# QMC-Cornell/sqmc

Measured on AMD Instinct MI355X. Metric: walker-steps/sec, higher is better.
Workload: dtype f64; 1 GPU; C2 cc-pVDZ r=1.24253 (8e,26o, D2h) semistochastic walk, uniform2 proposal, w_abs_gen_target=100000, size_deterministic=1000, Psi_T 100 dets, tau_multiplier 0.1, min_wt 0.5, r_initiator 1; rng=counter, parallelism=single GPU, devices=1, chained_runs=True

## Files before the change

### sqmc_amd/csrc/bucket_kernels.h

```cpp
#pragma once

__global__ void __launch_bounds__(BK_T) k_bucket_boundaries(const u64 *__restrict__ keys, long long n0, BucketArgs ba) { bk_rebalance_block(ba, keys, n0); }
__global__ void __launch_bounds__(BK_T) k_bucket_partition(const u64 *__restrict__ keys, long long n0, long long nch, u64 invalid_key, BucketArgs ba, int n_extra) {
  if ((int)blockIdx.x < n_extra) { bk_rebalance_block(ba, keys, n0); return; }
  __shared__ u32 spl[BK_MAXB];
  __shared__ u32 wcnt[BK_T / 64][BK_MAXB];
  const long long blk = (long long)blockIdx.x - n_extra;
  const long long c = blk * BK_T + threadIdx.x;
  u64 word = 0; u32 key = 0; bool valid = false;
  if (c < nch) word = keys[n0 + c];
  bucket_partition_stage(spl, &wcnt[0][0], BK_MAXB, keys, n0, ba);
  if (c < nch) { key = (u32)(word >> 32); valid = (u64)key != invalid_key; }
  __syncthreads();
  bucket_partition_block(spl, &wcnt[0][0], BK_MAXB, valid, key, word, blk, ba);
}

__device__ __forceinline__ void bk_fold(double &wt, int &ini, int &d, double w2, u32 fs, const StepP &p) {
  const int i2 = flg_init(fs), d2 = flg_impd(fs);
  const bool same_sign = (w2 * wt > 0);
  if (same_sign) { if (i2 > ini) ini = i2; }
  if (d == -2) { if (d2 == 0) d = 0; }
  else if (d2 == -2) { if (d != 0) d = -2; }
  else if (d != 0 && d != -2) { const int a_ = d2 < 0 ? -d2 : d2; if (a_ < d) d = a_; }
  if (!same_sign) {
    if (fabs(wt) < fabs(w2)) { if (ini != 3 || p.r_init == -1.0) ini = i2; }
    else if (fabs(wt) == fabs(w2)) { if (ini != 3 || p.r_init == -1.0) ini = 0; }
  }
  if (!(d == 0 && d2 == -1)) wt = wt + w2;
}

#ifdef BUCKET_PROF
__device__ unsigned long long g_bprof[16 * 1024];
#define BPROF(K) do { if (threadIdx.x == 0 && b < 1024) g_bprof[b * 16 + (K)] = wall_clock64(); } while (0)
#define BPROF_VAL(K, V) do { if (threadIdx.x == 0 && b < 1024) g_bprof[b * 16 + (K)] = (unsigned long long)(V); } while (0)
extern "C" int sqmc_gpu_debug_bprof(unsigned long long *out) { return (int)hipMemcpyFromSymbol(out, HIP_SYMBOL(g_bprof), sizeof(g_bprof)); }
#else
#define BPROF(K)
#define BPROF_VAL(K, V)
#endif
__device__ __forceinline__ u64 bk_block_excl_scan(u64 v, u64 *total) {
  __shared__ u64 wsum[BK_AT / 64];
  const int lane = threadIdx.x & 63, wv = threadIdx.x >> 6;
  const u64 inc = wave_incl_scan_u64(v, lane);
  if (lane == 63) wsum[wv] = inc;
  __syncthreads();
  u64 off = 0, tot = 0;
#pragma unroll
  for (int i = 0; i < BK_AT / 64; i++) { if (i < wv) off += wsum[i]; tot += wsum[i]; }
  __syncthreads();
  *total = tot;
  return off + inc - v;
}
__device__ __forceinline__ u64 bk_lookback_wide(u64 *__restrict__ state, int b, u64 tot) {
  __shared__ int s_pstar[BK_AT / 64]; __shared__ u64 s_part[BK_AT / 64];
  const int tid = threadIdx.x, lane = tid & 63, wv = tid >> 6;
  if (b == 0) { if (tid == 0) atomicExch((unsigned long long *)&state[0], SCAN_ST_INC | tot); return 0; }
  if (tid == 0) atomicExch((unsigned long long *)&state[b], SCAN_ST_AGG | tot);
  u64 w_[BK_MAXB / BK_AT]; int ix_[BK_MAXB / BK_AT];
  int pstar = -1;
#pragma unroll
  for (int q = 0; q < BK_MAXB / BK_AT; q++) {
    const int idx = b - 1 - tid - q * BK_AT; ix_[q] = idx; w_[q] = 0;
    if (idx >= 0) {
      u64 w;
      do { w = atomicAdd((unsigned long long *)&state[idx], 0ull); } while ((w >> 62) == 0);
      w_[q] = w;
      if ((w >> 62) == 2 && idx > pstar) pstar = idx;
    }
  }
  for (int o = 32; o > 0; o >>= 1) { const int x = __shfl_xor(pstar, o, 64); pstar = x > pstar ? x : pstar; }
  if (lane == 0) s_pstar[wv] = pstar;
  __syncthreads();
#pragma unroll
  for (int v = 0; v < BK_AT / 64; v++) pstar = s_pstar[v] > pstar ? s_pstar[v] : pstar;
  u64 sum = 0;
#pragma unroll
  for (int q = 0; q < BK_MAXB / BK_AT; q++) if (ix_[q] >= 0 && ix_[q] >= pstar) sum += w_[q] & SCAN_VAL_MASK;
  for (int o = 32; o > 0; o >>= 1) sum += __shfl_xor(sum, o, 64);
  if (lane == 0) s_part[wv] = sum;
  __syncthreads();
  u64 excl = 0;
#pragma unroll
  for (int v = 0; v < BK_AT / 64; v++) excl += s_part[v];
  if (tid == 0) atomicExch((unsigned long long *)&state[b], SCAN_ST_INC | (excl + tot));
  return excl;
}
#define BK_LONG_RUN 24
#define BK_LONG_MAX 32
#define BK_HQ_DETS (BK_CAP_T * 2 / 16)
template <int CTRL, int ROWMASK>
__device__ __forceinline__ double bk_dpp_f64(double v) {
  int lo = __double2loint(v), hi = __double2hiint(v);
  lo = __builtin_amdgcn_update_dpp(0, lo, CTRL, ROWMASK, 0xf, true);
  hi = __builtin_amdgcn_update_dpp(0, hi, CTRL, ROWMASK, 0xf, true);
  return __hiloint2double(hi, lo);
}
__device__ __forceinline__ double bk_wave_sum_lane63(double v) {
  v += bk_dpp_f64<0x111, 0xf>(v); v += bk_dpp_f64<0x112, 0xf>(v); v += bk_dpp_f64<0x114, 0xf>(v); v += bk_dpp_f64<0x118, 0xf>(v);
  v += bk_dpp_f64<0x142, 0xa>(v);
  v += bk_dpp_f64<0x143, 0xc>(v);
  return v;
}
#define BK_PER_ROWS ((BK_CAP_ROWS + BK_AT - 1) / BK_AT)
#define BK_PER_S ((BK_CAP_S + BK_AT - 1) / BK_AT)
#define BK_PER_R ((BK_CAP_R + BK_AT - 1) / BK_AT)
#define BK_PER_T ((BK_CAP_T + BK_AT - 1) / BK_AT)

__global__ void __launch_bounds__(BK_AT, BK_PER_CU * (BK_AT / 64) / 4) k_anneal_bucket(WalkArr w, WalkArr o, const u64 *__restrict__ rkeys, int *__restrict__ loc_imp,
                                                         const u64 *__restrict__ hkey, const u32 *__restrict__ hidx, u64 hmask,
                                                         const double *__restrict__ cnum, const double *__restrict__ cden,
                                                         double *__restrict__ partials, double *__restrict__ wabs_part, long long n0, long long nch, StepP p,
                                                         u64 invalid_key, u64 seed, u64 step, DevScalars *sc, BucketArgs ba, GateOut go, FusedSide fs, ChemDev dev) {
  __shared__ u64 sw[BK_CAP_S], sw2[BK_CAP_S];
  __shared__ u32 rk[BK_CAP_R];
  __shared__ double s_w[BK_CAP_T]; __shared__ u32 s_f[BK_CAP_T];
  __shared__ u32 m2s[BK_CAP_T];
  __shared__ __align__(16) unsigned short rnk[BK_CAP_T];
  constexpr int BK_SCR_TAB = (BK_CAP_T + 3) & ~3;
  constexpr int BK_SCR_ROWS = (BK_CAP_ROWS / 2 + 4) + BK_CAP_ROWS + 1, BK_SCR_CNT = (BK_AT / 64) * 1024 * (int)sizeof(bk_cnt_t) / 4, BK_SCR_TABEND = BK_SCR_TAB + ((int)sizeof(ChemTab) + 3) / 4;
  constexpr int BK_SCR_WORDS = ((BK_SCR_ROWS > BK_SCR_CNT ? (BK_SCR_ROWS > BK_SCR_TABEND ? BK_SCR_ROWS : BK_SCR_TABEND) : (BK_SCR_CNT > BK_SCR_TABEND ? BK_SCR_CNT : BK_SCR_TABEND)) + 3) & ~3;
  __shared__ __align__(16) u32 scratch[BK_SCR_WORDS];
  __shared__ unsigned short s_hq[BK_CAP_T]; __shared__ int s_hqn;
  static_assert(BK_CAP_T <= 4096 && (sizeof(bk_cnt_t) == 4 || BK_CAP_S <= 65535), "ranks inside a bucket are 12 bits; the counters hold a bucket's spawns");
  ChemTab *s_tab = (ChemTab *)(scratch + BK_SCR_TAB);
  u64 *s_hdet = (u64 *)rnk;
  __shared__ u32 s_tile; __shared__ u32 s_kmin, s_kmax;
  __shared__ double s_red[BK_AT / 64][NSTAT + 2];
  const int tid = threadIdx.x, lane = tid & 63, wv = tid >> 6;
  if (tid == 0) { s_tile = atomicAdd(ba.ticket, 1u); s_hqn = 0; }
  __syncthreads();
  const int b = (int)s_tile, B = ba.B, nsb = ba.nsb;
  const long long r_lo = bk_bound(ba, b, n0), r_hi = bk_bound(ba, b + 1, n0);
  const int R = (int)(r_hi - r_lo);
  BPROF(0);
  if (tid == 0) s_kmin = b ? (ba.kb ? ba.kb[b] : (u32)(rkeys[r_lo] >> 32)) : 0u;
  if (tid == 64) s_kmax = (b + 1 < B) ? (ba.kb ? ba.kb[b + 1] : (u32)(rkeys[r_hi] >> 32)) - 1u : (u32)invalid_key;
  unsigned short *seg_lo = (unsigned short *)scratch; u32 *seg_base = scratch + (BK_CAP_ROWS / 2 + 4);
  bool fits = nsb <= BK_CAP_ROWS && R <= BK_CAP_R && !(ba.kb && (b == 0 || b == B - 1) && R == 0);
  u32 rk_reg[BK_PER_R];
#pragma unroll
  for (int q = 0; q < BK_PER_R; q++) { const int i = tid + q * BK_AT; rk_reg[q] = (fits && i < R) ? (u32)(rkeys[r_lo + i] >> 32) : 0u; }
  int S = 0;
  const bool rows_ok = nsb <= BK_CAP_ROWS;
  if (rows_ok) {
    const int C = (nsb + BK_AT - 1) / BK_AT;
    unsigned short lo_[BK_PER_ROWS], hi_[BK_PER_ROWS];
#pragma unroll
    for (int q = 0; q < BK_PER_ROWS; q++) {
      const int t = tid * C + q;
      lo_[q] = 0; hi_[q] = 0;
      if (q < C && t < nsb) { const unsigned short *rp = ba.segoff + (long long)t * (B + 1) + b; lo_[q] = rp[0]; hi_[q] = rp[1]; }
    }
    u64 mine = 0;
#pragma unroll
    for (int q = 0; q < BK_PER_ROWS; q++) mine += (u64)(hi_[q] - lo_[q]);
    u64 tot; u32 ex = (u32)bk_block_excl_scan(mine, &tot);
#pragma unroll
    for (int q = 0; q < BK_PER_ROWS; q++) {
      const int t = tid * C + q;
      if (q < C && t < nsb) { seg_lo[t] = lo_[q]; seg_base[t] = ex; ex += (u32)(hi_[q] - lo_[q]); }
    }
    if (tid == 0) seg_base[nsb] = (u32)tot;
    S = (int)tot;
    fits = fits && S <= BK_CAP_S && R + S <= BK_CAP_T && !ba.force_retry;
  }
  const int T = R + S;
  if (!fits) {
    if (tid == 0) atomicExch((int *)&sc->retry, 1);
    if (tid == 0 && ba.scount && rows_ok) { ba.scount[b] = (u32)S; if (b == 0) ba.scount[B] = (u32)n0; }
#ifdef BUCKET_PROF
    if (tid == 0) printf("bucket %d of %d does not fit: rows %d, R %d, S %d (r_lo %lld)\n", b, B, nsb, R, S, r_lo);
#endif
    if (tid < 64) lookback_exclusive(ba.state, (u32)b, 0ull, tid);
    return;
  }
#pragma unroll
  for (int q = 0; q < BK_PER_R; q++) { const int i = tid + q * BK_AT; if (i < R) rk[i] = rk_reg[q]; }
  __syncthreads();
  BPROF(1);
  {
    u64 wv_[BK_PER_S];
#pragma unroll
    for (int q = 0; q < BK_PER_S; q++) {
      const int j = tid + q * BK_AT;
      wv_[q] = 0;
      if (j < S) {
        int lo = 0, hi = nsb;
        while (hi - lo > 1) { const int mid = (lo + hi) >> 1; if (seg_base[mid] <= (u32)j) lo = mid; else hi = mid; }
        wv_[q] = ba.words[(long long)lo * BK_T + seg_lo[lo] + ((u32)j - seg_base[lo])];
      }
    }
#pragma unroll
    for (int q = 0; q < BK_PER_S; q++) { const int j = tid + q * BK_AT; if (j < S) sw[j] = wv_[q]; }
  }
  __syncthreads();
  BPROF(2); BPROF_VAL(12, S); BPROF_VAL(13, R);
  if (tid == 0 && ba.scount) { ba.scount[b] = (u32)S; if (b == 0) ba.scount[B] = (u32)n0; }
  u64 *sa = sw, *sb = sw2;
  const bool gap_sort = R <= 1023;
  unsigned short *gs = (unsigned short *)m2s, *gst = gs + BK_CAP_S;
  static_assert((BK_CAP_S + 1026) * 2 <= BK_CAP_T * 4, "gap tables fit the merged-order array");
  if (gap_sort) {
    unsigned short *gp = s_hq;
    bk_cnt_t(*wcnt)[1024] = (bk_cnt_t(*)[1024])scratch;
    const u64 lt = (lane == 0) ? 0ull : (~0ull >> (64 - lane));
    const int chunk = ((S + BK_AT - 1) / BK_AT) * 64;
    for (int d = tid; d < BK_SCR_CNT; d += BK_AT) scratch[d] = 0;
    for (int j = tid; j < S; j += BK_AT) {
      const u32 k = (u32)(sa[j] >> 32);
      int lo = 0, hi = R;
      while (lo < hi) { const int mid = (lo + hi) >> 1; if (rk[mid] <= k) lo = mid + 1; else hi = mid; }
      gp[j] = (unsigned short)lo;
    }
    __syncthreads();
    {
      const int beg = wv * chunk, end = (beg + chunk < S) ? beg + chunk : S;
      for (int base = beg; base < end; base += 64) {
        const int idx = base + lane; const bool valid = idx < end;
        const u32 dig = valid ? (u32)gp[idx] : 0u;
        u64 same = __ballot(valid);
#pragma unroll
        for (int q = 0; q < 10; q++) { const u64 m = __ballot((dig >> q) & 1); same &= ((dig >> q) & 1) ? m : ~m; }
        const u32 rank = (u32)__popcll(same & lt), cnt = (u32)__popcll(same);
        u32 prev = 0;
        if (valid) prev = wcnt[wv][dig];
        __builtin_amdgcn_wave_barrier();
        if (valid && rank == 0) wcnt[wv][dig] = (bk_cnt_t)(prev + cnt);
        __builtin_amdgcn_wave_barrier();
        if (valid) rnk[idx] = (unsigned short)(prev + rank);
      }
    }
    __syncthreads();
    {
      u32 t2[2]; u64 sum = 0;
#pragma unroll
      for (int q = 0; q < 2; q++) { const int d = tid * 2 + q; u32 s2 = 0; for (int v = 0; v < BK_AT / 64; v++) s2 += wcnt[v][d]; t2[q] = s2; sum += s2; }
      u64 tt; u32 ex = (u32)bk_block_excl_scan(sum, &tt);
#pragma unroll
      for (int q = 0; q < 2; q++) {
        const int d = tid * 2 + q; u32 a2 = ex;
        if (d <= R) gst[d] = (unsigned short)ex;
        for (int v = 0; v < BK_AT / 64; v++) { const u32 cn = wcnt[v][d]; wcnt[v][d] = (bk_cnt_t)a2; a2 += cn; }
        ex += t2[q];
      }
      if (tid == 0) gst[R + 1] = (unsigned short)S;
    }
    __syncthreads();
    for (int idx = tid; idx < S; idx += BK_AT) {
      const u32 dig = (u32)gp[idx];
      const u32 pos = wcnt[idx / chunk][dig] + rnk[idx];
      sb[pos] = sa[idx]; gs[pos] = (unsigned short)dig;
    }
    __syncthreads();
    for (int j = tid; j < S; j += BK_AT) {
      const u64 mine = sb[j];
      const int g0 = (int)gs[j], a2 = (int)gst[g0], e2 = (int)gst[g0 + 1];
      int less = 0;
      if (e2 - a2 > 1) for (int i = a2; i < e2; i++) less += (sb[i] < mine) ? 1 : 0;
      sa[a2 + less] = mine;
    }
    __syncthreads();
  } else {
  {
    const u32 kmin = s_kmin, span = s_kmax - kmin;
    int nbits = 0; while (nbits < 32 && (span >> nbits)) nbits++;
    const int npass = (nbits + 9) / 10, dbits = npass ? (nbits + npass - 1) / npass : 0;
    const int chunk = ((S + BK_AT - 1) / BK_AT) * 64;
    bk_cnt_t(*wcnt)[1024] = (bk_cnt_t(*)[1024])scratch;
    const u64 lt = (lane == 0) ? 0ull : (~0ull >> (64 - lane));
    for (int ps = 0, shift = 0; ps < npass && S > 1; ps++, shift += dbits) {
      const u32 mask = (1u << dbits) - 1u;
      for (int d = tid; d < BK_SCR_CNT; d += BK_AT) scratch[d] = 0;
      __syncthreads();
      const int beg = wv * chunk, end = (beg + chunk < S) ? beg + chunk : S;
      for (int base = beg; base < end; base += 64) {
        const int idx = base + lane; const bool valid = idx < end;
        const u32 dig = valid ? ((((u32)(sa[idx] >> 32) - kmin) >> shift) & mask) : 0u;
        u64 same = __ballot(valid);
        for (int q = 0; q < dbits; q++) { const u64 m = __ballot((dig >> q) & 1); same &= ((dig >> q) & 1) ? m : ~m; }
        const u32 rank = (u32)__popcll(same & lt), cnt = (u32)__popcll(same);
        u32 prev = 0;
        if (valid) prev = wcnt[wv][dig];
        __builtin_amdgcn_wave_barrier();
        if (valid && rank == 0) wcnt[wv][dig] = (bk_cnt_t)(prev + cnt);
        __builtin_amdgcn_wave_barrier();
        if (valid) rnk[idx] = (unsigned short)(prev + rank);
      }
      __syncthreads();
      {
        u32 t2[2]; u64 sum = 0;
#pragma unroll
        for (int q = 0; q < 2; q++) { const int d = tid * 2 + q; u32 s2 = 0; for (int v = 0; v < BK_AT / 64; v++) s2 += wcnt[v][d]; t2[q] = s2; sum += s2; }
        u64 tt; u32 ex = (u32)bk_block_excl_scan(sum, &tt);
#pragma unroll
        for (int q = 0; q < 2; q++) { const int d = tid * 2 + q; u32 a = ex; for (int v = 0; v < BK_AT / 64; v++) { const u32 cn = wcnt[v][d]; wcnt[v][d] = (bk_cnt_t)a; a += cn; } ex += t2[q]; }
      }
      __syncthreads();
      for (int idx = tid; idx < S; idx += BK_AT) {
        const u64 x = sa[idx];
        const u32 dig = ((((u32)(x >> 32)) - kmin) >> shift) & mask;
        sb[wcnt[idx / chunk][dig] + rnk[idx]] = x;
      }
      __syncthreads();
      u64 *tp = sa; sa = sb; sb = tp;
    }
  }
  }
  BPROF(3);
  {
    double rw[BK_PER_R]; u32 rf[BK_PER_R]; double rm[BK_PER_R]; u32 rr[BK_PER_R]; double sw_[BK_PER_S]; u64 sf_[BK_PER_S];
#pragma unroll
    for (int q = 0; q < BK_PER_R; q++) {
      const int i = tid + q * BK_AT; rw[q] = 0.0; rf[q] = 0; rm[q] = 0.0; rr[q] = 0;
      if (i < R) { rw[q] = w.wt[r_lo + i]; rf[q] = w.flg[r_lo + i]; if (fs.on) { rm[q] = w.me[r_lo + i]; rr[q] = w.irk[r_lo + i]; } }
    }
#pragma unroll
    for (int q = 0; q < BK_PER_S; q++) {
      const int j = tid + q * BK_AT; sw_[q] = 0.0; sf_[q] = 0;
      if (j < S) { const SpawnRec *rp = w.sp + ((long long)(u32)sa[j] - n0); sw_[q] = rp->wt; sf_[q] = rp->flg; }
    }
#pragma unroll
    for (int q = 0; q < BK_PER_R; q++) {
      const int i = tid + q * BK_AT;
      if (i < R) {
        double x = rw[q];
        if (fs.on) {
          const int impd = flg_impd(rf[q]);
          if (!(p.semi && impd < 1)) {
            double f = 1.0 + p.tau * (p.e_trial - rm[q]);
            if (f < 0) { if (p.reached > 1) sc->err = SQMC_ERR_NEG_DIAG; f = 0; }
            x = x * f;
          } else if (impd == 0) {
            double y = fs.y[rr[q]];
            y = y + p.e_trial * p.tau * fs.x_in[rr[q]];
            x = x + y;
          }
        }
        s_w[i] = x; s_f[i] = rf[q];
      }
    }
#pragma unroll
    for (int q = 0; q < BK_PER_S; q++) { const int j = tid + q * BK_AT; if (j < S) { s_w[R + j] = sw_[q]; s_f[R + j] = (u32)sf_[q]; } }
  }
  __syncthreads();
  BPROF(4);
  double wabs = 0.0, cnt = 0.0;
  for (int x = tid; x < T; x += BK_AT) { wabs += fabs(s_w[x]); cnt += 1.0; }
  if (gap_sort) {
    u32 rp_[BK_PER_R], cp_[BK_PER_S]; u32 ce_[BK_PER_S];
#pragma unroll
    for (int q = 0; q < BK_PER_R; q++) { const int i = tid + q * BK_AT; rp_[q] = (i < R) ? (u32)i + (u32)gst[i + 1] : 0u; }
#pragma unroll
    for (int q = 0; q < BK_PER_S; q++) {
      const int j = tid + q * BK_AT; cp_[q] = 0; ce_[q] = 0;
      if (j < S) {
        const u32 k = (u32)(sa[j] >> 32); const int g0 = (int)gs[j];
        const bool on_resident = g0 > 0 && rk[g0 - 1] == k;
        const bool head = !on_resident && (j == 0 || (u32)(sa[j - 1] >> 32) != k);
        cp_[q] = (u32)(j + g0); ce_[q] = (head ? BK_STOP : 0u) | (u32)(R + j);
      }
    }
    __syncthreads();
#pragma unroll
    for (int q = 0; q < BK_PER_R; q++) { const int i = tid + q * BK_AT; if (i < R) m2s[rp_[q]] = BK_STOP | (u32)i; }
#pragma unroll
    for (int q = 0; q < BK_PER_S; q++) { const int j = tid + q * BK_AT; if (j < S) m2s[cp_[q]] = ce_[q]; }
  } else {
  for (int i = tid; i < R; i += BK_AT) {
    const u32 k = rk[i];
    int lo = 0, hi = S;
    while (lo < hi) { const int mid = (lo + hi) >> 1; if ((u32)(sa[mid] >> 32) < k) lo = mid + 1; else hi = mid; }
    m2s[i + lo] = BK_STOP | (u32)i;
  }
  for (int j = tid; j < S; j += BK_AT) {
    const u32 k = (u32)(sa[j] >> 32);
    int lo = 0, hi = R;
    while (lo < hi) { const int mid = (lo + hi) >> 1; if (rk[mid] <= k) lo = mid + 1; else hi = mid; }
    const bool on_resident = lo > 0 && rk[lo - 1] == k;
    const bool head = !on_resident && (j == 0 || (u32)(sa[j - 1] >> 32) != k);
    m2s[j + lo] = (head ? BK_STOP : 0u) | (u32)(R + j);
  }
  }
  __syncthreads();
  BPROF(5);
  u32 *s_nc = scratch;
  auto finish_head = [&](int q, int si, double wt, int ini, int d, int psg, int qq) -> unsigned short {
    unsigned short keep = 0;
    {
      const int dd = d - p.imind > 0 ? d - p.imind : 0;
      const double thr = p.r_init * ipow_d(dd, p.ipow), aw = fabs(wt);
      if (ini == 3 && p.r_init >= 0) { if (wt * psg < 1.0) wt = (double)psg; }
      else if (ini == 2 && ((aw <= thr && d > 0) || ((aw <= p.r_init && !p.cti) && d == -2))) ini = 1;
      else if (ini < 2 && ((aw > thr && d >= 0) || ((aw > p.r_init || p.cti) && d == -2))) ini = ini + 1;
    }
    int dtest = d;
    if (d == -1) { if (b == B - 1 && qq >= T) dtest = 1; d = 1; }
    const bool discard = (((wt == 0.0 && (ini != 3 || p.r_init < 0)) || ini == 0) && dtest >= 1);
    if (!discard) {
      if (d >= 1 && fabs(wt) < p.min_wt) {
        const u32 kk = (si < R) ? rk[si] : (u32)(sa[si - R] >> 32);
        Rng g; g.mode = 1; g.x = sq_counter_key(seed, step, 2, (u64)kk);
        if (rng_draw(g) < (fabs(wt) / p.min_wt)) wt = copysign(p.min_wt, wt); else wt = 0.0;
      }
      if (!(wt == 0.0 && d >= 1)) keep = (d == 0) ? 0x101 : 0x1;
    }
    s_w[si] = wt; s_f[si] = pack_flg(d, ini, psg);
    if (go.child_off && keep) {
      const u32 kk = (si < R) ? rk[si] : (u32)(sa[si - R] >> 32);
      u64 nc; double wc;
      gate_children(wt * p.rfi, go.cutoff, seed, go.step_next, (u64)kk, nc, wc);
      s_nc[q] = (u32)nc;
    }
    return keep;
  };
  __shared__ int s_lq[BK_LONG_MAX], s_lqq[BK_LONG_MAX], s_lini[BK_LONG_MAX], s_ld[BK_LONG_MAX], s_nlong;
  __shared__ double s_lwt[BK_LONG_MAX];
  if (tid == 0) s_nlong = 0;
  __syncthreads();
  for (int q = tid; q < T; q += BK_AT) {
    const u32 e = m2s[q];
    unsigned short keep = 0;
    if (e & BK_STOP) {
      const int si = (int)(e & ~BK_STOP);
      double wt = s_w[si]; const u32 f0 = s_f[si];
      int ini = flg_init(f0), d = flg_impd(f0); const int psg = flg_psign(f0);
      if (d == -1 && !(b == 0 && q == 0)) d = 1;
      int qq = q + 1;
      bool more = false;
      for (; qq < T; qq++) {
        const u32 e2 = m2s[qq];
        if (e2 & BK_STOP) break;
        if (qq - q > BK_LONG_RUN) { more = true; break; }
        bk_fold(wt, ini, d, s_w[e2], s_f[e2], p);
      }
      int slot = -1;
      if (more) { slot = atomicAdd(&s_nlong, 1); if (slot >= BK_LONG_MAX) { slot = -1; for (; qq < T; qq++) { const u32 e2 = m2s[qq]; if (e2 & BK_STOP) break; bk_fold(wt, ini, d, s_w[e2], s_f[e2], p); } } }
      if (slot >= 0) { s_lq[slot] = q; s_lqq[slot] = qq; s_lwt[slot] = wt; s_lini[slot] = ini; s_ld[slot] = d; }
      else keep = finish_head(q, si, wt, ini, d, psg, qq);
    }
    rnk[q] = keep;
  }
  __syncthreads();
  {
    const int nlong = s_nlong < BK_LONG_MAX ? s_nlong : BK_LONG_MAX;
    for (int k = wv; k < nlong; k += BK_AT / 64) {
      const int q = s_lq[k]; int qq = s_lqq[k];
      double wt = s_lwt[k]; int ini = s_lini[k], d = s_ld[k];
      const int si = (int)(m2s[q] & ~BK_STOP);
      const int psg = flg_psign(s_f[si]);
      const bool keep3 = !(p.r_init == -1.0);
      for (;;) {
        const int idx = qq + lane;
        const u32 e2 = (idx < T) ? m2s[idx] : BK_STOP;
        const u64 stops = __ballot((e2 & BK_STOP) != 0);
        const int n = stops ? (int)__builtin_ctzll(stops) : 64;
        if (n > 0) {
          const bool in = lane < n;
          const int e0 = (int)(__shfl((int)(e2 & ~BK_STOP), 0, 64));
          const double w2 = in ? s_w[e0 + lane] : 0.0; const u32 f2 = in ? s_f[e0 + lane] : 0u;
          const int i2 = flg_init(f2), d2 = flg_impd(f2);
          const u64 skipm = __ballot(in && d == 0 && d2 == -1);
          const bool anym2 = __ballot(in && d2 == -2) != 0ull;
          int am = (in && d2 != -2) ? (d2 < 0 ? -d2 : d2) : 0x7FFFFFFF;
          __builtin_amdgcn_wave_barrier();
          if (lane == 0) {
            double run = wt;
            int z = 0;
            for (; z + 8 <= n; z += 8) {
              double a_[8];
#pragma unroll
              for (int y = 0; y < 8; y++) a_[y] = s_w[e0 + z + y];
#pragma unroll
              for (int y = 0; y < 8; y++) { s_w[e0 + z + y] = run; if (!((skipm >> (z + y)) & 1ull)) run = run + a_[y]; }
            }
            for (; z < n; z++) { const double wz = s_w[e0 + z]; s_w[e0 + z] = run; if (!((skipm >> z) & 1ull)) run = run + wz; }
            wt = run;
          }
          __builtin_amdgcn_wave_barrier();
          const double wb = in ? s_w[e0 + lane] : 0.0;
          u32 tab = 0xE4u;
          if (in) {
            if (w2 * wb > 0.0) { tab = 0; for (int x = 0; x < 4; x++) tab |= (u32)(x > i2 ? x : i2) << (2 * x); }
            else if (fabs(wb) < fabs(w2)) { tab = 0; for (int x = 0; x < 4; x++) tab |= (u32)((x != 3 || !keep3) ? i2 : x) << (2 * x); }
            else if (fabs(wb) == fabs(w2)) { tab = 0; for (int x = 0; x < 4; x++) tab |= (u32)((x != 3 || !keep3) ? 0 : x) << (2 * x); }
          }
          for (int o = 1; o < 64; o <<= 1) {
            const u32 nxt = (u32)__shfl_down((int)tab, o, 64);
            const int am2 = __shfl_down(am, o, 64);
            if (lane + o < 64) {
              u32 c2 = 0;
              for (int x = 0; x < 4; x++) c2 |= ((nxt >> (2 * ((tab >> (2 * x)) & 3u))) & 3u) << (2 * x);
              tab = c2;
              am = am2 < am ? am2 : am;
            }
          }
          tab = (u32)__shfl((int)tab, 0, 64); am = __shfl(am, 0, 64);
          ini = (int)((tab >> (2 * ini)) & 3u);
          if (d != 0 && d != -2) { if (anym2) d = -2; else if (d != -1 && am < d) d = am; }
          wt = __shfl(wt, 0, 64);
          qq += n;
        }
        if (stops) break;
      }
      if (lane == 0) rnk[q] = finish_head(q, si, wt, ini, d, psg, qq);
    }
  }
  __syncthreads();
  BPROF(6);
  u32 *s_rank = (u32 *)sb;
  u64 ex_glob;
  {
    const int C = (T + BK_AT - 1) / BK_AT, beg = tid * C, end = (beg + C < T) ? beg + C : T;
    const bool ch = go.child_off != nullptr;
    u64 mine = 0;
    for (int q = beg; q < end; q++) { const unsigned short k = rnk[q]; if (k & 1) mine += 1ull | ((u64)(k >> 8) << 20) | (ch ? ((u64)s_nc[q] << 38) : 0ull); }
    u64 tot; u64 ex = bk_block_excl_scan(mine, &tot);
    for (int q = beg; q < end; q++) {
      const unsigned short k = rnk[q];
      if (k & 1) {
        s_rank[q] = (u32)(ex & 0xFFFull) | ((u32)((ex >> 20) & 0x3FFFFull) << 12);
        const u64 add = 1ull | ((u64)(k >> 8) << 20) | (ch ? ((u64)s_nc[q] << 38) : 0ull);
        if (ch) s_nc[q] = (u32)(ex >> 38);
        ex += add;
      } else s_rank[q] = 0xFFFFFFFFu;
    }
    __syncthreads();
    stage_tab(s_tab, dev.tab, dev.tab_words);
    ex_glob = bk_lookback_wide(ba.state, b, tot);
    if (tid == 0 && b == B - 1) {
      const u64 all = ex_glob + tot, npos = all & 0xFFFFFull, ndet = (all >> 20) & 0x3FFFFull;
      sc->tot2 = npos | (ndet << 32); sc->nwalk = npos;
      if (ch) sc->n_children = all >> 38;
    }
    BPROF(9);
  }
  BPROF(7);
  double st[NSTAT];
#pragma unroll
  for (int k = 0; k < NSTAT; k++) st[k] = 0.0;
  constexpr int CB = 2;
  for (int q0b = tid; q0b < T; q0b += CB * BK_AT) {
    int si_[CB]; u32 r_[CB]; u64 up_[CB], dn_[CB], key_[CB]; double me_[CB], en_[CB], ed_[CB]; long long hh_[CB];
#pragma unroll
    for (int z = 0; z < CB; z++) {
      const int q = q0b + z * BK_AT;
      r_[z] = (q < T) ? s_rank[q] : 0xFFFFFFFFu;
      si_[z] = 0; up_[z] = 0; dn_[z] = 0; key_[z] = 0; me_[z] = 1e51; en_[z] = 1e51; ed_[z] = 1e51; hh_[z] = -2;
      if (r_[z] != 0xFFFFFFFFu) {
        const int si = (int)(m2s[q] & ~BK_STOP); si_[z] = si;
        if (si < R) { const long long ix = r_lo + si; up_[z] = w.up[ix]; dn_[z] = w.dn[ix]; me_[z] = w.me[ix]; en_[z] = w.en[ix]; ed_[z] = w.ed[ix]; key_[z] = rk[si]; }
        else { const u64 x = sa[si - R]; const SpawnRec *rp = w.sp + ((long long)(u32)x - n0); up_[z] = rp->up; dn_[z] = rp->dn; key_[z] = x >> 32; }
      }
    }
#pragma unroll
    for (int z = 0; z < CB; z++) if (r_[z] != 0xFFFFFFFFu && en_[z] > 1e50) hh_[z] = ct_lookup(hkey, hidx, hmask, key_[z]);
#pragma unroll
    for (int z = 0; z < CB; z++) if (hh_[z] != -2) { if (hh_[z] < 0) { en_[z] = 0.0; ed_[z] = 0.0; } else { en_[z] = cnum[hh_[z]]; ed_[z] = cden[hh_[z]]; } }
#pragma unroll
    for (int z = 0; z < CB; z++) {
      if (r_[z] == 0xFFFFFFFFu) continue;
      const int si = si_[z];
      const long long q0 = (long long)(ex_glob & 0xFFFFFull) + (long long)(r_[z] & 0xFFFu);
      const long long qd = (long long)((ex_glob >> 20) & 0x3FFFFull) + (long long)(r_[z] >> 12);
      const double wt = s_w[si] * p.rfi;
      const u32 fl = s_f[si];
      const int d = flg_impd(fl), ini = flg_init(fl), psg = flg_psign(fl);
      const double en = en_[z], ed = ed_[z];
      o.up[q0] = up_[z]; o.dn[q0] = dn_[z]; o.wt[q0] = wt; o.flg[q0] = fl;
      o.me[q0] = me_[z]; o.en[q0] = en; o.ed[q0] = ed;
      if (me_[z] > 1e50 && !(p.semi && d < 1)) {
        const int slot = atomicAdd(&s_hqn, 1);
        s_hq[slot] = (unsigned short)(r_[z] & 0xFFFu);
        if (slot < BK_HQ_DETS) { s_hdet[2 * slot] = up_[z]; s_hdet[2 * slot + 1] = dn_[z]; }
      }
      if (go.on) {
        u64 nc; double wc;
        gate_children(wt, go.cutoff, seed, go.step_next, key_[z], nc, wc);
        go.keys[q0] = (key_[z] << 32) | (u64)q0; go.wchild[q0] = wc;
        if (go.child_off) { const u64 off = (ex_glob >> 38) + (u64)s_nc[q0b + z * BK_AT]; go.child_off[q0] = off; gate_block_parents(go.bpar, off, nc, q0); } else go.nchild[q0] = nc;
      }
      if (d == 0 && p.semi && qd < p.nimp_cap) { loc_imp[qd] = (int)q0; o.irk[q0] = (u32)qd; if (fs.x_out) fs.x_out[qd] = wt; }
      st[0] += wt; st[1] += fabs(wt); st[8] += wt * wt;
      if (ini == 3) st[4] += wt * psg;
      if (d == 0 || (d == -2 && p.cti)) st[6] += fabs(wt);
      double e_num = en * wt, e_den = ed * wt;
      if (e_num != 0.0) {
        if (fabs(e_den) < 1e-22) e_den = fabs(e_den);
        st[2] += e_den; st[3] += e_num; st[9] += e_num * e_num; st[10] += e_den * e_den;
        st[11] += e_num * copysign(1.0, e_den); st[12] += fabs(e_den); st[5] += e_num * e_den;
      }
    }
  }
  BPROF(8);
  __syncthreads();
  BPROF(14);
  {
    const int nq = s_hqn;
    BPROF_VAL(15, nq);
    const long long base = (long long)(ex_glob & 0xFFFFFull);
    const int hg = bk_hii_group_lanes(*s_tab);
    int n_def = 0;
    if (ba.hq_cnt) {
      n_def = nq < BK_HQ_DEFER ? nq : BK_HQ_DEFER;
      for (int k = tid; k < n_def; k += BK_AT) ba.hq_pos[b * BK_HQ_DEFER + k] = (u32)(base + (long long)s_hq[k]);
      if (tid == 0) ba.hq_cnt[b] = (u32)n_def;
    }
#define BK_HII_PASSES(HG)                                                                                          \
    {                                                                                                              \
      const int G = tid / HG, g = tid % HG;                                                                        \
      double *sg = s_w + G * BK_HG_TERMS(HG);                    \
      for (int k0 = n_def; k0 < nq; k0 += BK_AT / HG) {                                                            \
        const int k = k0 + G; const bool valid = k < nq;                                                           \
        const long long q0 = valid ? base + (long long)s_hq[k] : 0;                                                \
        u64 u = 0, dd = 0;                                                                                         \
        if (valid) { if (k < BK_HQ_DETS) { u = s_hdet[2 * k]; dd = s_hdet[2 * k + 1]; } else { u = o.up[q0]; dd = o.dn[q0]; } }   \
        const double v = bk_hii_group<HG>(*s_tab, dev.integrals, u, dd, valid, sg, g);                             \
        if (valid && g == 0) o.me[q0] = v;                                                                         \
      }                                                                                                            \
    }
    if (nq == n_def) { }
    else if ((hg == 8 || hg == 16) && nq - n_def <= BK_AT / 32 && bk_hii_terms(*s_tab) <= BK_HG_TERMS(32)) BK_HII_PASSES(32)
    else if (hg == 8 && nq - n_def <= BK_AT / 16) BK_HII_PASSES(16)
    else if (hg == 8) BK_HII_PASSES(8)
    else if (hg == 16) BK_HII_PASSES(16)
    else {
      for (int k = n_def + tid; k < nq; k += BK_AT) {
        const long long q0 = base + (long long)s_hq[k];
        const u64 u = o.up[q0], dd = o.dn[q0];
        o.me[q0] = h_any(*s_tab, dev.integrals, u, dd, u, dd);
      }
    }
#undef BK_HII_PASSES
  }
  BPROF(11);
#pragma unroll
  for (int k = 0; k < NSTAT + 2; k++) {
    double v = (k < NSTAT) ? st[k] : (k == NSTAT ? wabs : cnt);
    v = bk_wave_sum_lane63(v);
    if (lane == 63) s_red[wv][k] = v;
  }
  __syncthreads();
  if (tid < NSTAT + 2) {
    double v = 0.0;
    for (int q = 0; q < BK_AT / 64; q++) v += s_red[q][tid];
    if (tid < NSTAT) partials[(long long)b * NSTAT + tid] = v;
    else wabs_part[2 * b + (tid - NSTAT)] = v;
  }
  BPROF(10);
  if (tid == 0) { const int fs = (1000 * S) / BK_CAP_S, ft = (1000 * T) / BK_CAP_T; atomicMax((unsigned int *)&sc->bk_fill, (unsigned int)(fs > ft ? fs : ft)); }
}
```

Measured before the change: 2.052 billion walker-steps/s.

## Prefetch resident and spawn records before bucket sort and scatter via permutation

Resident walker fields (weight, flags, energy, index) and the deterministic-space y/x values are now loaded into registers at the top of the bucket kernel, before the sort. Short spawn rows (up to eight words in the first few row slots per thread) are fetched directly alongside the segment offsets, and the binary-search gather runs only when wide rows exist. Spawn records are read in unsorted order while the sort is in progress. The sort tracks a permutation so the loaded values can be scattered to their sorted slots afterwards. The aim is to overlap global-memory latency with the sort, at the cost of more registers (possibly lower occupancy) and extra index bookkeeping in shared memory.

After: 2.012 billion walker-steps/s. -2.0%, worse.

```diff
diff --git a/sqmc_amd/csrc/bucket_kernels.h b/sqmc_amd/csrc/bucket_kernels.h
--- a/sqmc_amd/csrc/bucket_kernels.h
+++ b/sqmc_amd/csrc/bucket_kernels.h
@@ -105,6 +105,8 @@
 #define BK_PER_S ((BK_CAP_S + BK_AT - 1) / BK_AT)
 #define BK_PER_R ((BK_CAP_R + BK_AT - 1) / BK_AT)
 #define BK_PER_T ((BK_CAP_T + BK_AT - 1) / BK_AT)
+#define BK_ROW_Q (BK_PER_ROWS < 3 ? BK_PER_ROWS : 3)
+#define BK_ROW_W 8
 
 __global__ void __launch_bounds__(BK_AT, BK_PER_CU * (BK_AT / 64) / 4) k_anneal_bucket(WalkArr w, WalkArr o, const u64 *__restrict__ rkeys, int *__restrict__ loc_imp,
                                                          const u64 *__restrict__ hkey, const u32 *__restrict__ hidx, u64 hmask,
@@ -138,9 +140,19 @@
   unsigned short *seg_lo = (unsigned short *)scratch; u32 *seg_base = scratch + (BK_CAP_ROWS / 2 + 4);
   bool fits = nsb <= BK_CAP_ROWS && R <= BK_CAP_R && !(ba.kb && (b == 0 || b == B - 1) && R == 0);
   u32 rk_reg[BK_PER_R];
-#pragma unroll
-  for (int q = 0; q < BK_PER_R; q++) { const int i = tid + q * BK_AT; rk_reg[q] = (fits && i < R) ? (u32)(rkeys[r_lo + i] >> 32) : 0u; }
-  int S = 0;
+  double rw[BK_PER_R]; u32 rf[BK_PER_R]; double rm[BK_PER_R]; u32 rr[BK_PER_R];
+#pragma unroll
+  for (int q = 0; q < BK_PER_R; q++) {
+    const int i = tid + q * BK_AT; rk_reg[q] = 0u; rw[q] = 0.0; rf[q] = 0; rm[q] = 0.0; rr[q] = 0;
+    if (fits && i < R) {
+      rk_reg[q] = (u32)(rkeys[r_lo + i] >> 32); rw[q] = w.wt[r_lo + i]; rf[q] = w.flg[r_lo + i];
+      if (fs.on) { rm[q] = w.me[r_lo + i]; rr[q] = w.irk[r_lo + i]; }
+    }
+  }
+  int S = 0, n_wide = 0;
+  u64 wr_[BK_ROW_Q][BK_ROW_W]; u32 wr_at[BK_ROW_Q]; int wr_n[BK_ROW_Q];
+#pragma unroll
+  for (int q = 0; q < BK_ROW_Q; q++) { wr_at[q] = 0; wr_n[q] = 0; }
   const bool rows_ok = nsb <= BK_CAP_ROWS;
   if (rows_ok) {
     const int C = (nsb + BK_AT - 1) / BK_AT;
@@ -151,17 +163,26 @@
       lo_[q] = 0; hi_[q] = 0;
       if (q < C && t < nsb) { const unsigned short *rp = ba.segoff + (long long)t * (B + 1) + b; lo_[q] = rp[0]; hi_[q] = rp[1]; }
     }
+#pragma unroll
+    for (int q = 0; q < BK_ROW_Q; q++) {
+      const int t = tid * C + q, n = (int)hi_[q] - (int)lo_[q];
+#pragma unroll
+      for (int i = 0; i < BK_ROW_W; i++) { wr_[q][i] = 0; if (n <= BK_ROW_W && i < n) wr_[q][i] = ba.words[(long long)t * BK_T + lo_[q] + i]; }
+    }
     u64 mine = 0;
 #pragma unroll
-    for (int q = 0; q < BK_PER_ROWS; q++) mine += (u64)(hi_[q] - lo_[q]);
-    u64 tot; u32 ex = (u32)bk_block_excl_scan(mine, &tot);
+    for (int q = 0; q < BK_PER_ROWS; q++) { const u32 n = (u32)(hi_[q] - lo_[q]); mine += (u64)n + ((n > 0 && (q >= BK_ROW_Q || n > BK_ROW_W)) ? (1ull << 32) : 0ull); }
+    u64 tot; const u64 ex64 = bk_block_excl_scan(mine, &tot);
+    u32 ex = (u32)ex64;
 #pragma unroll
     for (int q = 0; q < BK_PER_ROWS; q++) {
       const int t = tid * C + q;
-      if (q < C && t < nsb) { seg_lo[t] = lo_[q]; seg_base[t] = ex; ex += (u32)(hi_[q] - lo_[q]); }
+      if (q < C && t < nsb) { seg_lo[t] = lo_[q]; seg_base[t] = ex; if (q < BK_ROW_Q) wr_at[q] = ex; ex += (u32)(hi_[q] - lo_[q]); }
     }
     if (tid == 0) seg_base[nsb] = (u32)tot;
-    S = (int)tot;
+    S = (int)(u32)tot; n_wide = (int)(tot >> 32);
+#pragma unroll
+    for (int q = 0; q < BK_ROW_Q; q++) wr_n[q] = ((int)hi_[q] - (int)lo_[q] <= BK_ROW_W) ? (int)hi_[q] - (int)lo_[q] : 0;
     fits = fits && S <= BK_CAP_S && R + S <= BK_CAP_T && !ba.force_retry;
   }
   const int T = R + S;
@@ -176,32 +197,51 @@
   }
 #pragma unroll
   for (int q = 0; q < BK_PER_R; q++) { const int i = tid + q * BK_AT; if (i < R) rk[i] = rk_reg[q]; }
+  double ry[BK_PER_R], rx[BK_PER_R];
+#pragma unroll
+  for (int q = 0; q < BK_PER_R; q++) {
+    const int i = tid + q * BK_AT; ry[q] = 0.0; rx[q] = 0.0;
+    if (fs.on && p.semi && i < R && flg_impd(rf[q]) == 0) { ry[q] = fs.y[rr[q]]; rx[q] = fs.x_in[rr[q]]; }
+  }
+#pragma unroll
+  for (int q = 0; q < BK_ROW_Q; q++) {
+#pragma unroll
+    for (int i = 0; i < BK_ROW_W; i++) if (i < wr_n[q]) sw[wr_at[q] + i] = wr_[q][i];
+  }
   __syncthreads();
   BPROF(1);
-  {
-    u64 wv_[BK_PER_S];
+  if (n_wide) {
+    const int C = (nsb + BK_AT - 1) / BK_AT;
+    u64 wv_[BK_PER_S]; bool wide[BK_PER_S];
 #pragma unroll
     for (int q = 0; q < BK_PER_S; q++) {
       const int j = tid + q * BK_AT;
-      wv_[q] = 0;
+      wv_[q] = 0; wide[q] = false;
       if (j < S) {
         int lo = 0, hi = nsb;
         while (hi - lo > 1) { const int mid = (lo + hi) >> 1; if (seg_base[mid] <= (u32)j) lo = mid; else hi = mid; }
-        wv_[q] = ba.words[(long long)lo * BK_T + seg_lo[lo] + ((u32)j - seg_base[lo])];
-      }
-    }
-#pragma unroll
-    for (int q = 0; q < BK_PER_S; q++) { const int j = tid + q * BK_AT; if (j < S) sw[j] = wv_[q]; }
-  }
-  __syncthreads();
+        wide[q] = (lo % C) >= BK_ROW_Q || seg_base[lo + 1] - seg_base[lo] > (u32)BK_ROW_W;
+        if (wide[q]) wv_[q] = ba.words[(long long)lo * BK_T + seg_lo[lo] + ((u32)j - seg_base[lo])];
+      }
+    }
+#pragma unroll
+    for (int q = 0; q < BK_PER_S; q++) { const int j = tid + q * BK_AT; if (wide[q]) sw[j] = wv_[q]; }
+    __syncthreads();
+  }
+  double sw_[BK_PER_S]; u64 sf_[BK_PER_S];
+#pragma unroll
+  for (int q = 0; q < BK_PER_S; q++) {
+    const int j = tid + q * BK_AT; sw_[q] = 0.0; sf_[q] = 0;
+    if (j < S) { const SpawnRec *rp = w.sp + ((long long)(u32)sw[j] - n0); sw_[q] = rp->wt; sf_[q] = rp->flg; }
+  }
   BPROF(2); BPROF_VAL(12, S); BPROF_VAL(13, R);
   if (tid == 0 && ba.scount) { ba.scount[b] = (u32)S; if (b == 0) ba.scount[B] = (u32)n0; }
   u64 *sa = sw, *sb = sw2;
   const bool gap_sort = R <= 1023;
   unsigned short *gs = (unsigned short *)m2s, *gst = gs + BK_CAP_S;
   static_assert((BK_CAP_S + 1026) * 2 <= BK_CAP_T * 4, "gap tables fit the merged-order array");
+  unsigned short *gp = s_hq;
   if (gap_sort) {
-    unsigned short *gp = s_hq;
     bk_cnt_t(*wcnt)[1024] = (bk_cnt_t(*)[1024])scratch;
     const u64 lt = (lane == 0) ? 0ull : (~0ull >> (64 - lane));
     const int chunk = ((S + BK_AT - 1) / BK_AT) * 64;
@@ -250,6 +290,7 @@
       const u32 dig = (u32)gp[idx];
       const u32 pos = wcnt[idx / chunk][dig] + rnk[idx];
       sb[pos] = sa[idx]; gs[pos] = (unsigned short)dig;
+      gp[idx] = (unsigned short)pos;
     }
     __syncthreads();
     for (int j = tid; j < S; j += BK_AT) {
@@ -258,6 +299,7 @@
       int less = 0;
       if (e2 - a2 > 1) for (int i = a2; i < e2; i++) less += (sb[i] < mine) ? 1 : 0;
       sa[a2 + less] = mine;
+      rnk[j] = (unsigned short)(a2 + less);
     }
     __syncthreads();
   } else {
@@ -268,6 +310,9 @@
     const int chunk = ((S + BK_AT - 1) / BK_AT) * 64;
     bk_cnt_t(*wcnt)[1024] = (bk_cnt_t(*)[1024])scratch;
     const u64 lt = (lane == 0) ? 0ull : (~0ull >> (64 - lane));
+    unsigned short *pa = (unsigned short *)m2s, *pb = pa + BK_CAP_S;
+    static_assert(BK_CAP_S * 2 * 2 <= BK_CAP_T * 4, "two index arrays fit the merged-order array");
+    bool moved = false;
     for (int ps = 0, shift = 0; ps < npass && S > 1; ps++, shift += dbits) {
       const u32 mask = (1u << dbits) - 1u;
       for (int d = tid; d < BK_SCR_CNT; d += BK_AT) scratch[d] = 0;
@@ -299,26 +344,19 @@
       for (int idx = tid; idx < S; idx += BK_AT) {
         const u64 x = sa[idx];
         const u32 dig = ((((u32)(x >> 32)) - kmin) >> shift) & mask;
-        sb[wcnt[idx / chunk][dig] + rnk[idx]] = x;
+        const u32 np = wcnt[idx / chunk][dig] + rnk[idx];
+        sb[np] = x; pb[np] = moved ? pa[idx] : (unsigned short)idx;
       }
       __syncthreads();
       u64 *tp = sa; sa = sb; sb = tp;
-    }
+      unsigned short *tq = pa; pa = pb; pb = tq; moved = true;
+    }
+    for (int j = tid; j < S; j += BK_AT) { if (moved) gp[pa[j]] = (unsigned short)j; else gp[j] = (unsigned short)j; }
+    __syncthreads();
   }
   }
   BPROF(3);
   {
-    double rw[BK_PER_R]; u32 rf[BK_PER_R]; double rm[BK_PER_R]; u32 rr[BK_PER_R]; double sw_[BK_PER_S]; u64 sf_[BK_PER_S];
-#pragma unroll
-    for (int q = 0; q < BK_PER_R; q++) {
-      const int i = tid + q * BK_AT; rw[q] = 0.0; rf[q] = 0; rm[q] = 0.0; rr[q] = 0;
-      if (i < R) { rw[q] = w.wt[r_lo + i]; rf[q] = w.flg[r_lo + i]; if (fs.on) { rm[q] = w.me[r_lo + i]; rr[q] = w.irk[r_lo + i]; } }
-    }
-#pragma unroll
-    for (int q = 0; q < BK_PER_S; q++) {
-      const int j = tid + q * BK_AT; sw_[q] = 0.0; sf_[q] = 0;
-      if (j < S) { const SpawnRec *rp = w.sp + ((long long)(u32)sa[j] - n0); sw_[q] = rp->wt; sf_[q] = rp->flg; }
-    }
 #pragma unroll
     for (int q = 0; q < BK_PER_R; q++) {
       const int i = tid + q * BK_AT;
@@ -331,8 +369,8 @@
             if (f < 0) { if (p.reached > 1) sc->err = SQMC_ERR_NEG_DIAG; f = 0; }
             x = x * f;
           } else if (impd == 0) {
-            double y = fs.y[rr[q]];
-            y = y + p.e_trial * p.tau * fs.x_in[rr[q]];
+            double y = ry[q];
+            y = y + p.e_trial * p.tau * rx[q];
             x = x + y;
           }
         }
@@ -340,7 +378,10 @@
       }
     }
 #pragma unroll
-    for (int q = 0; q < BK_PER_S; q++) { const int j = tid + q * BK_AT; if (j < S) { s_w[R + j] = sw_[q]; s_f[R + j] = (u32)sf_[q]; } }
+    for (int q = 0; q < BK_PER_S; q++) {
+      const int j = tid + q * BK_AT;
+      if (j < S) { const int f = gap_sort ? (int)rnk[gp[j]] : (int)gp[j]; s_w[R + f] = sw_[q]; s_f[R + f] = (u32)sf_[q]; }
+    }
   }
   __syncthreads();
   BPROF(4);
```
